# BUTSpeechFIT/VBx

Measured on NVIDIA H100. Metric: x-vectors/sec through 10 VB-HMM EM iters, higher is better.
Workload: dtype f32

## Files before the change

vbx_b200/csrc/vbx_kernels.cu:

```cuda
#include <math_constants.h>

#include "vbx_internal.cuh"

namespace vbx {

__device__ __forceinline__ void cp_async16(void *smem, const void *gmem) {
    unsigned s = static_cast<unsigned>(__cvta_generic_to_shared(smem));
    asm volatile("cp.async.cg.shared.global [%0], [%1], 16;\n" ::"r"(s), "l"(gmem));
}
__device__ __forceinline__ void cp_async_wait_all() {
    asm volatile("cp.async.commit_group;\n" ::);
    asm volatile("cp.async.wait_group 0;\n" ::: "memory");
}

template <int LANES>
__device__ __forceinline__ float group_sum(float v) {
#pragma unroll
    for (int off = LANES / 2; off > 0; off >>= 1) v += __shfl_xor_sync(0xffffffffu, v, off);
    return v;
}
template <int LANES>
__device__ __forceinline__ float group_max(float v) {
#pragma unroll
    for (int off = LANES / 2; off > 0; off >>= 1) v = fmaxf(v, __shfl_xor_sync(0xffffffffu, v, off));
// ... 324 lines not shown
    }
    const int R4 = R >> 2;
    float *out = ws.partial + (int64_t)tile * S_PAD * R;
    for (int i = threadIdx.x; i < S_PAD * R4; i += 256) {
        const int s = i / R4, c4 = i - s * R4;
        *reinterpret_cast<float4 *>(out + (int64_t)s * R + 4 * c4) = *reinterpret_cast<const float4 *>(&red[s][4 * c4]);
    }
}

int launch_mstep_partial(const Plan &pl, const Workspace &ws, const float *rho, const float *gamma, cudaStream_t st) {
    if (pl.n_mtiles == 0) return 0;
    switch (pl.S) {
        case 4: mstep_partial_kernel<4><<<pl.n_mtiles, 256, 0, st>>>(pl, ws, rho, gamma); break;
        case 8: mstep_partial_kernel<8><<<pl.n_mtiles, 256, 0, st>>>(pl, ws, rho, gamma); break;
        case 16: mstep_partial_kernel<16><<<pl.n_mtiles, 256, 0, st>>>(pl, ws, rho, gamma); break;
        case 32: mstep_partial_kernel<32><<<pl.n_mtiles, 256, 0, st>>>(pl, ws, rho, gamma); break;
        case 64: mstep_partial_kernel<64><<<pl.n_mtiles, 256, 0, st>>>(pl, ws, rho, gamma); break;
        case kMaxSWide: {
            constexpr int smem = kMaxSWide * kMaxR * sizeof(float);
            static bool configured = false;
            if (!configured) {
                if (cudaFuncSetAttribute(mstep_partial_kernel<kMaxSWide>, cudaFuncAttributeMaxDynamicSharedMemorySize, smem) != cudaSuccess)
                    return -1;
                configured = true;
            }
            mstep_partial_kernel<kMaxSWide><<<pl.n_mtiles, 256, smem, st>>>(pl, ws, rho, gamma);
            break;
        }
        default: return -1;
    }
    return cudaGetLastError() == cudaSuccess ? 1 : -1;
}

template <int S8, bool R128>
__global__ void __launch_bounds__(512) speaker_model_kernel(Plan pl, Workspace ws, const float *__restrict__ Phi,
                                                            const int32_t *__restrict__ n_states, float *alpha_io,
                                                            float *invL_io, int from_given) {
    const int S = pl.S, R = pl.R;
    constexpr int NT = S8 / 8, NSP = S8 / 4;
    const int rec = blockIdx.x;
    if (!ws.active[rec]) return;
    const float FaFb = ws.hp[rec].FaFb, Fa = ws.hp[rec].Fa;
    const int wg = threadIdx.x >> 7;
    const int r = threadIdx.x & 127, warp = r >> 5, lane = r & 31;
    const bool live = r < R;
    const int ns = n_states ? n_states[rec] : S;
    const float phi = live ? Phi[r] : 0.f;
    const int t_lo = pl.mtile_begin[rec], t_hi = pl.mtile_begin[rec + 1];
    extern __shared__ float sAv[];
    __shared__ double cpart[S8 > kMaxS ? S8 : kMaxS][4], rpart[S8 > kMaxS ? S8 : kMaxS][4];
    constexpr int NCH = NSP < 16 ? NSP : 16;
#pragma unroll
    for (int k0 = 0; k0 < NSP; k0 += NCH) {
    double grs[NCH];
#pragma unroll
    for (int k = 0; k < NCH; ++k) {
        const int s = wg + 4 * (k0 + k);
        double gr = 0.0;
        if (live && s < ns && !from_given)
            for (int t = t_lo; t < t_hi; ++t) gr += (double)__ldg(ws.partial + ((int64_t)t * S + s) * R + r);
        grs[k] = gr;
    }
#pragma unroll
    for (int k = 0; k < NCH; ++k) {
        const int s = wg + 4 * (k0 + k);
        const int64_t o = ((int64_t)rec * S + s) * R + r;
        const bool dead = s >= ns;
        float invL = 1.f, alpha = 0.f, Av = 0.f;
        float c = 0.f, reg = 0.f;
        if (live && !dead) {
            if (from_given) {
                alpha = alpha_io[o];
                invL = invL_io[o];
            } else {
                const double gr = grs[k];
                const float Ns = ws.occ[(int64_t)rec * S + s];
                invL = 1.f / (1.f + FaFb * Ns * phi);
                alpha = (float)((double)(FaFb * invL) * gr);
            }
            Av = Fa * alpha;
            const float a2 = alpha * alpha;
            reg = logf(invL) - invL - a2 + 1.f;
            c = (invL + a2) * phi;
        }
        if (live && s < S) {
            ws.A[o] = Av;
            if (!from_given || dead) {
                if (alpha_io) alpha_io[o] = dead ? 0.f : alpha;
                if (invL_io) invL_io[o] = dead ? 0.f : invL;
            }
        }
        sAv[s * kMaxR + r] = Av;
        c = group_sum<32>(c);
        reg = group_sum<32>(reg);
        if (lane == 0) {
            cpart[s][warp] = (double)c;
            rpart[s][warp] = (double)reg;
        }
    }
    }
    __syncthreads();
    if (threadIdx.x < S) {
        const int s = threadIdx.x;
        const bool dead = s >= ns;
        ws.bias[(int64_t)rec * S + s] =
            dead ? CUDART_INF_F : (float)(ws.hp[rec].dFa * 0.5 * ((cpart[s][0] + cpart[s][1]) + (cpart[s][2] + cpart[s][3])));
        ws.regp[(int64_t)rec * S + s] = dead ? 0.0 : (rpart[s][0] + rpart[s][1]) + (rpart[s][2] + rpart[s][3]);
    }
    const int KS = R128 ? 16 : (R + 7) >> 3, KQ = 2 * KS;
    float *fh = ws.Afrag_hi + (int64_t)rec * NT * KS * 64, *fl = ws.Afrag_lo + (int64_t)rec * NT * KS * 64;
    for (int q = threadIdx.x; q < NT * KS * 64; q += 512) {
        const int e = q & 1, ln = (q >> 1) & 31, ij = q >> 6;
        const int j = R128 ? (ij & 15) : ij % KS, i = R128 ? (ij >> 4) : ij / KS;
        const int st = 8 * i + (ln >> 2), fq = ln & 3;
        const int col = R128 ? 16 * (j >> 1) + 4 * fq + 2 * (j & 1) + e : KQ * fq + 2 * j + e;
        const float Av = col < kMaxR ? sAv[st * kMaxR + col] : 0.f;
        const float hi = __uint_as_float(__float_as_uint(Av) & 0xffffe000u);
        fh[q] = hi;
        fl[q] = Av - hi;
    }
}

int launch_speaker_model(const Plan &pl, const Workspace &ws, const float *Phi,
                         const int32_t *n_states, float *alpha_io, float *invL_io, bool from_given,
                         cudaStream_t st) {
    if (pl.n_rec == 0) return 0;
    const int S8 = pl.S > 8 ? pl.S : 8;
    const size_t smem = (size_t)S8 * kMaxR * sizeof(float);
    const int fg = from_given ? 1 : 0;
    if (S8 == kMaxSWide) {
        static bool configured = false;
        if (!configured) {
            if (cudaFuncSetAttribute(speaker_model_kernel<kMaxSWide, true>, cudaFuncAttributeMaxDynamicSharedMemorySize, (int)smem) != cudaSuccess ||
                cudaFuncSetAttribute(speaker_model_kernel<kMaxSWide, false>, cudaFuncAttributeMaxDynamicSharedMemorySize, (int)smem) != cudaSuccess)
                return -1;
            configured = true;
        }
    }
#define VBX_SM(S8_, R_) speaker_model_kernel<S8_, R_><<<pl.n_rec, 512, smem, st>>>(pl, ws, Phi, n_states, alpha_io, invL_io, fg)
    if (pl.R == 128) {
        switch (S8) {
            case 8: VBX_SM(8, true); break;
            case 16: VBX_SM(16, true); break;
            case 32: VBX_SM(32, true); break;
            case kMaxSWide: VBX_SM(kMaxSWide, true); break;
            default: VBX_SM(64, true); break;
        }
    } else {
        switch (S8) {
            case 8: VBX_SM(8, false); break;
            case 16: VBX_SM(16, false); break;
            case 32: VBX_SM(32, false); break;
            case kMaxSWide: VBX_SM(kMaxSWide, false); break;
            default: VBX_SM(64, false); break;
        }
    }
#undef VBX_SM
    return cudaGetLastError() == cudaSuccess ? 1 : -1;
}

template <int S_PAD>
__global__ void __launch_bounds__(128) loglik_kernel(Plan pl, Workspace ws, const float *__restrict__ rho,
                                                     const float *__restrict__ pi, const int32_t *__restrict__ n_states) {
    constexpr int SL = S_PAD < 8 ? S_PAD : 8;
    constexpr int SJ = S_PAD / SL;
    constexpr int FL = 128 / SL;
    constexpr int FJ = kLTile / FL;
    extern __shared__ float4 smem4[];
    float *smem = reinterpret_cast<float *>(smem4);
    const int R = pl.R, RP = R + 4, R4 = R >> 2;
    float *rhoS = smem;
    float *AS = smem + kLTile * RP;
    const int tile = blockIdx.x;
    const int rec = pl.ltile_rec[tile];
    if (!ws.active[rec]) return;
    const int64_t f0 = pl.ltile_f0[tile];
    const int len = (int)min((int64_t)kLTile, pl.offsets[rec + 1] - f0);
    const int tid = threadIdx.x;
    {
        const float *src = rho + f0 * R;
        for (int i = tid; i < len * R4; i += 128) {
            const int row = i / R4, c4 = i - row * R4;
            cp_async16(rhoS + row * RP + 4 * c4, src + (int64_t)row * R + 4 * c4);
        }
        const float *Ab = ws.A + (int64_t)rec * S_PAD * R;
        for (int i = tid; i < S_PAD * R4; i += 128) {
            const int row = i / R4, c4 = i - row * R4;
            cp_async16(AS + row * RP + 4 * c4, Ab + (int64_t)row * R + 4 * c4);
// ... 662 lines not shown
    for (int k = 0; k < SPL; ++k) {
        ys[k] = (st.rn * ps.v[k]) * fmaf(P, st.y[k], w[k] * st.Yc);
        locq = fmaf(pn.v[k], ys[k], locq);
        locc = fmaf(pn.v[k], w[k], locc);
    }
    const float qn = group_sum<LPR>(locq);
    const float cn = group_sum<LPR>(locc);
    const float Ys = st.rn * fmaf(P, st.q, st.c * st.Yc);
    const float inv = rcp_fast(Ys);
    const float rsig = st.rn * st.Yc * inv;
#pragma unroll
    for (int k = 0; k < SPL; ++k) {
        an[k] = ys[k] * inv;
        st.y[k] = ys[k];
    }
    st.Yc = Ys;
    st.q = qn;
    st.c = cn;
    st.rn = st.rs1;
    st.rs1 = rsig;
    return rsig;
}

template <int S_PAD, int SPL>
struct FbRing {
    static constexpr int LPR = S_PAD / SPL, RPW = 32 / LPR;
    static constexpr int F = (SPL == 4) ? 5 : (SPL == 2 ? 10 : 16);
    static constexpr int FF = 2 * F;
    static constexpr int RW = (F + 6 + 3) / 4 * 4;
    static constexpr int GROUP = 2 * F * S_PAD + RW;
    static constexpr int STAGE = RPW * GROUP;
    static constexpr int kStages = 3;
    static constexpr int kSmemBytes = 128 + 4 * kStages * STAGE * 4;
};

template <int S_PAD, int SPL>
__global__ void __launch_bounds__(128) forward_backward_ring_kernel(Plan pl, Workspace ws, RunParams rp, float *gamma,
                                                                    float *pi_io, const int32_t *__restrict__ n_states) {
    using G = FbRing<S_PAD, SPL>;
    constexpr int LPR = G::LPR, RPW = G::RPW, F = G::F, FF = G::FF, NST = G::kStages;
    extern __shared__ __align__(128) unsigned char fb_ring_smem[];
    const int lane = threadIdx.x & 31, warp = threadIdx.x >> 5;
    const int warp_global = blockIdx.x * 4 + warp;
    const int g = lane / LPR, l = lane % LPR;
    const int slot = warp_global * RPW + g;
    int rec = -1;
    if (slot < pl.n_rec) rec = pl.order[slot];
    const bool live = rec >= 0 && ws.active[rec] != 0 && pl.lrec_nchunks[rec] == 0;
    int64_t f0 = 0;
    int T = 0;
    if (live) {
        f0 = pl.offsets[rec];
        T = (int)(pl.offsets[rec + 1] - f0);
    }
    int Tmax = T, Tmin = live ? T : 0x7fffffff;
#pragma unroll
    for (int off = 16; off > 0; off >>= 1) {
        Tmax = max(Tmax, __shfl_xor_sync(0xffffffffu, Tmax, off));
        Tmin = min(Tmin, __shfl_xor_sync(0xffffffffu, Tmin, off));
    }
    if (Tmax == 0) return;
    const int Tlast = max(T - 1, 0);
    const int ns = live ? (n_states ? n_states[rec] : S_PAD) : 0;
    const float P = rec >= 0 ? ws.hp[rec].loopP : 0.f, Q = 1.f - P;

    float pi[SPL], w[SPL];
#pragma unroll
    for (int k = 0; k < SPL; ++k) {
        const int s = l * SPL + k;
        const bool sl = live && s < ns;
// ... 159 lines not shown
            }
            {
                const float sc = rcp_fast(group_sum<LPR>(gs));
#pragma unroll
                for (int k = 0; k < SPL; ++k) gn[k] *= sc;
            }
            if (!check) {
#pragma unroll
                for (int k = 0; k < SPL; ++k) {
                    g0[k] = gn[k];
                    occf[k] += gn[k];
                    entf[k] += v[k];
                }
                sto_vec<SPL>(ga + t * gstr, gn);
            } else {
                const bool act = t >= 0;
#pragma unroll
                for (int k = 0; k < SPL; ++k) {
                    g0[k] = act ? gn[k] : g0[k];
                    occf[k] += act ? gn[k] : 0.f;
                    entf[k] += act ? v[k] : 0.f;
                }
                if (act) sto_vec<SPL>(ga + t * gstr, gn);
            }
#pragma unroll
            for (int k = 0; k < SPL; ++k) {
                b[k] = bn[k];
                kap[k] = kapn[k];
            }
            dprev = d;
            e = en;
            f = fn;
        };
        auto bstage = [&](const int u, const float *st, const int rb, const bool check) {
            const float *sp = st + l * SPL, *sr = st + 2 * F * S_PAD;
            const int lo = T - 1 - (u + 1) * F, z = min(max(-lo, 0), F - 1);
            Vec<SPL> pr[F];
            float rt[F];
#pragma unroll
            for (int i = 0; i < F; ++i) {
                pr[i] = ld_vec<SPL>(sp + i * S_PAD);
                rt[i] = sr[max(rb - i, 0)];
            }
            FwdState<SPL> fs, f1;
            {
                const Vec<SPL> cy = ld_vec<SPL>(sp + F * S_PAD);
                const Vec<4> c4 = ld_vec<4>(st + (F + 1) * S_PAD);
                const float crs = st[(F + 2) * S_PAD];
                const Vec<SPL> q0 = ld_vec<SPL>(sp + z * S_PAD), q1 = ld_vec<SPL>(sp + min(z + 1, F - 1) * S_PAD);
                if (u + NST - 1 < nb) issue_bwd(u + NST - 1);
                float a0[SPL];
                fwd_init<SPL, LPR>(f1, q0, q1, pi, w, l, live, ns, a0);
                const bool ck = lo >= 1;
#pragma unroll
                for (int k = 0; k < SPL; ++k) {
                    fs.y[k] = ck ? cy.v[k] : f1.y[k];
                    f1.y[k] = a0[k];
                }
                fs.Yc = ck ? c4.v[0] : f1.Yc;
                fs.q = ck ? c4.v[1] : f1.q;
                fs.c = ck ? c4.v[2] : f1.c;
                fs.rn = ck ? c4.v[3] : f1.rn;
                fs.rs1 = ck ? crs : f1.rs1;
            }
            Vec<SPL> a[F];
#pragma unroll
            for (int i = 0; i < F; ++i) {
                const int s = lo + i;
                FwdState<SPL> nx = fs;
                fwd_step<SPL, LPR>(nx, pr[i], pr[min(i + 1, F - 1)], w, P, a[i].v);
                if (s >= 1) fs = nx;
#pragma unroll
                for (int k = 0; k < SPL; ++k) a[i].v[k] = s == 0 ? f1.y[k] : a[i].v[k];
            }
#pragma unroll
            for (int i = 0; i < F; ++i) bstep(u * F + i, a[F - 1 - i], pr[F - 1 - i], rt[i], check);
#pragma unroll
            for (int k = 0; k < SPL; ++k) {
                occ[k] += (double)occf[k];
                enter[k] += (double)entf[k];
                occf[k] = 0.f;
                entf[k] = 0.f;
            }
        };
        for (int u = 0; u < nb; ++u) {
            mbar_wait(bar_of(nf + u), ((nf + u) / NST) & 1);
            const float *st = stage_of(nf + u);
            const int rb = (int)min((int64_t)(T - 2 - u * F) - rwin(u), (int64_t)(G::RW - 1));
            if ((u + 1) * F <= Tmin - 1)
                bstage(u, st, rb, false);
            else
                bstage(u, st, rb, true);
        }
    }

    double pn[SPL];
    float loc = 0.f;
#pragma unroll
    for (int k = 0; k < SPL; ++k) {
        pn[k] = (double)g0[k] + (double)Q * (double)pi[k] * enter[k];
        loc += (float)pn[k];
    }
    const float tot = group_sum<LPR>(loc);
    if (live) {
#pragma unroll
        for (int k = 0; k < SPL; ++k) {
            const int s = l * SPL + k;
            pi_io[(int64_t)rec * S_PAD + s] = (float)(pn[k] / (double)tot);
            ws.occ[(int64_t)rec * S_PAD + s] = (float)occ[k];
        }
    }
}

constexpr int64_t kRingMaxT = 2048;

template <int S_PAD, int SPL>
static int launch_fb_t(const Plan &pl, const Workspace &ws, const RunParams &rp, float *gamma, float *pi,
                       const int32_t *n_states, bool classic, bool ring, cudaStream_t st) {
    constexpr int RPW = 32 / (S_PAD / SPL);
    const int warps = (pl.n_rec + RPW - 1) / RPW;
    const int blocks = (warps + 3) / 4;
    if (classic) {
        forward_backward_kernel<S_PAD, SPL><<<blocks, 128, 0, st>>>(pl, ws, rp, gamma, pi, n_states);
    } else if (ring && pl.max_T <= kRingMaxT && (reinterpret_cast<uintptr_t>(gamma) & 15) == 0) {
        constexpr int smem = FbRing<S_PAD, SPL>::kSmemBytes;
        if (cudaFuncSetAttribute(forward_backward_ring_kernel<S_PAD, SPL>, cudaFuncAttributeMaxDynamicSharedMemorySize,
                                 smem) != cudaSuccess)
            return -1;
        forward_backward_ring_kernel<S_PAD, SPL><<<blocks, 128, smem, st>>>(pl, ws, rp, gamma, pi, n_states);
    } else {
        forward_backward_la_kernel<S_PAD, SPL><<<blocks, 128, 0, st>>>(pl, ws, rp, gamma, pi, n_states);
    }
    return cudaGetLastError() == cudaSuccess ? 1 : -1;
}

__global__ void __launch_bounds__(128) elbo_kernel(Plan pl, Workspace ws, RunParams rp, double *Li, int32_t *n_iters,
                                                   int32_t *flags, int iter) {
    const int rec = blockIdx.x;
    if (!ws.active[rec]) return;
    const int tid = threadIdx.x, lane = tid & 31, warp = tid >> 5;
    const int64_t f0 = pl.offsets[rec];
    const int T = (int)(pl.offsets[rec + 1] - f0);
    const float *rs = ws.rsigma + f0;
    const float *mx = ws.rowmax + f0;
    double acc = 0.0;
    for (int t = tid; t < T; t += 128) acc += (double)mx[t] - log((double)rs[t]);
    acc = warp_sum_d(acc);
// ... 124 lines not shown
```

vbx_b200/csrc/vbx_capi.cu:

```cuda
#include <dlfcn.h>
#include <nvtx3/nvToolsExt.h>

#include <algorithm>
#include <cmath>
#include <cstdio>
#include <cstring>
#include <numeric>
#include <string>
#include <vector>

#include "../../include/vbx_b200.h"
#include "vbx_internal.cuh"

struct vbx_handle_s {
    int device = 0;
    int sms = 0;
    std::string err;
    vbx::Plan plan;
    vbx::Workspace ws;
    bool planned = false, bound = false, prepared = false;
    bool f64_only = false;
    size_t ws_need = 0;
    void *plan_mem = nullptr;
    int opt_fb_spl = 0;
// ... 56 lines not shown
    }
    DeviceGuard(const DeviceGuard &) = delete;
    DeviceGuard &operator=(const DeviceGuard &) = delete;
};

struct Carver {
    char *base;
    size_t off = 0;
    explicit Carver(void *b) : base(static_cast<char *>(b)) {}
    template <typename T>
    T *take(size_t n) {
        T *p = base ? reinterpret_cast<T *>(base + off) : nullptr;
        off += align_up(n * sizeof(T));
        return p;
    }
};

void drop_graph(vbx_handle_t h) {
    if (h->graph_exec) cudaGraphExecDestroy(h->graph_exec);
    h->graph_exec = nullptr;
    h->graph_key = h->seen_key = 0;
}

size_t carve(const vbx::Plan &pl, void *base, vbx::Workspace *ws) {
    Carver c(base);
    const size_t N = (size_t)pl.n_frames, S = (size_t)pl.S, R = (size_t)pl.R, B = (size_t)pl.n_rec;
    vbx::Workspace w;
    w.p = c.take<float>(N * S);
    w.rowmax = c.take<float>(N);
    w.rsigma = c.take<float>(N);
    w.cvec = c.take<float>(N);
    w.partial = c.take<float>((size_t)pl.n_mtiles * S * R);
    w.A = c.take<float>(B * S * R);
    {
        const size_t NT = S > 8 ? S / 8 : 1, KS = (R + 7) / 8;
        w.Afrag_hi = c.take<float>(B * NT * KS * 64);
        w.Afrag_lo = c.take<float>(B * NT * KS * 64);
    }
    w.bias = c.take<float>(B * S);
    w.occ = c.take<float>(B * S);
    w.regp = c.take<double>(B * S);
    w.gsum = c.take<double>(B);
    w.gpart = c.take<double>((size_t)pl.n_mtiles);
    w.prev_elbo = c.take<double>(B);
    w.active = c.take<int32_t>(B);
    w.scratch = c.take<float>(2 * std::max<size_t>(S, vbx::kMaxS));
    if (pl.R == 128) w.tc_scratch = c.take<float>(vbx::tc_scratch_floats());
    if (pl.split) {
        w.ahat = c.take<float>(N * S);
        w.bhat = c.take<float>(N * S);
        w.socc = c.take<float>((size_t)pl.n_mtiles * S);
        w.sent = c.take<float>((size_t)pl.n_mtiles * S);
    }
    {
        const size_t LC = (size_t)pl.n_lchunks;
        w.fa_u = c.take<float>(LC * S * S);
        w.fa_lam = c.take<float>(LC * S);
        w.fa_exp = c.take<float>(LC * S);
        w.astart = c.take<float>(LC * S);
        w.bb_v = c.take<float>(LC * S * S);
        w.bb_mu = c.take<float>(LC * S);
        w.bb_exp = c.take<float>(LC * S);
        w.beta = c.take<float>(LC * S);
        w.occp = c.take<float>(LC * S);
        w.entp = c.take<float>(LC * S);
    }
    if (pl.exact) {
        w.active64 = c.take<int32_t>(B);
        w.fresh = c.take<int32_t>(B);
        w.gamma_snap = c.take<float>(2 * N * S);
        w.pi_snap = c.take<float>(2 * B * S);
// ... 1136 lines not shown
```

vbx_b200/csrc/vbx_internal.cuh:

```cuda
#pragma once
#include <cuda_runtime.h>
#include <stdint.h>

#include <string>
#include <vector>

#define VBX_EPS_TR 1e-8f

namespace vbx {

constexpr int kLTile = 64;
constexpr int kMTile = 512;
constexpr int kLongT = 4096;
constexpr int kChunk = 256;
constexpr int kMaxR = 128;
constexpr int kMaxS = 64;
constexpr int kMaxSWide = 128;
constexpr int kTcMaxD = 2048;

struct Plan {
    int32_t n_rec = 0, R = 0, S = 0;
    int32_t exact = 0;
    int32_t split = 0;
    int64_t n_frames = 0;
    int32_t n_ltiles = 0, n_mtiles = 0;
    int64_t max_T = 0;
    const int64_t *offsets = nullptr;
    const int32_t *order = nullptr;
    const int32_t *ltile_rec = nullptr;
    const int64_t *ltile_f0 = nullptr;
    const int32_t *mtile_rec = nullptr;
    const int64_t *mtile_f0 = nullptr;
    const int32_t *mtile_begin = nullptr;
    int32_t n_lrec = 0, n_lchunks = 0;
    const int32_t *lrec_list = nullptr;
    const int32_t *lrec_first = nullptr;
    const int32_t *lrec_nchunks = nullptr;
    const int32_t *lchunk_rec = nullptr;
    const int32_t *lchunk_idx = nullptr;
};

struct RecParams {
    float Fa, Fb, FaFb, loopP;
    double dFa, dFb, dFaFb, dloopP;
};

struct Workspace {
    float *p = nullptr;
    float *rowmax = nullptr;
    float *rsigma = nullptr;
    float *cvec = nullptr;
    float *partial = nullptr;
    float *A = nullptr;
    float *Afrag_hi = nullptr;
    float *Afrag_lo = nullptr;
    float *bias = nullptr;
    float *occ = nullptr;
    double *regp = nullptr;
    double *gsum = nullptr;
    double *gpart = nullptr;
    double *prev_elbo = nullptr;
    int32_t *active = nullptr;
    int32_t *active64 = nullptr;
    int32_t *fresh = nullptr;
    float *gamma_snap = nullptr;
    float *pi_snap = nullptr;
    double *p64 = nullptr;
    double *rowmax64 = nullptr;
    double *rsig64 = nullptr;
    double *partial64 = nullptr;
    double *occp64 = nullptr;
    double *alpha64 = nullptr;
    double *bias64 = nullptr;
    double *reg64 = nullptr;
    double *pi64 = nullptr;
    float *scratch = nullptr;
    float *ahat = nullptr, *bhat = nullptr;
    float *socc = nullptr, *sent = nullptr;
    float *tc_scratch = nullptr;
    float *fa_u = nullptr, *fa_lam = nullptr, *fa_exp = nullptr, *astart = nullptr;
    float *bb_v = nullptr, *bb_mu = nullptr, *bb_exp = nullptr, *beta = nullptr;
    float *occp = nullptr, *entp = nullptr;
    RecParams *hp = nullptr;
};

struct RunParams {
    double epsilon;
    int32_t max_iters;
// ... 242 lines not shown
```

vbx_b200/csrc/vbx_mma_kernels.cu:

```cuda
#include <math_constants.h>

#include "vbx_internal.cuh"

namespace vbx {

__device__ __forceinline__ void mma_tf32(float (&d)[4], const uint32_t (&a)[4], const uint32_t b0, const uint32_t b1) {
    asm volatile(
        "mma.sync.aligned.m16n8k8.row.col.f32.tf32.tf32.f32 {%0,%1,%2,%3}, {%4,%5,%6,%7}, {%8,%9}, {%0,%1,%2,%3};\n"
        : "+f"(d[0]), "+f"(d[1]), "+f"(d[2]), "+f"(d[3])
        : "r"(a[0]), "r"(a[1]), "r"(a[2]), "r"(a[3]), "r"(b0), "r"(b1));
}
__device__ __forceinline__ void split_tf32(const float x, uint32_t &hi, uint32_t &lo) {
    asm volatile("{\n\t.reg .b32 t;\n\tadd.u32 t, %1, 0x1000;\n\tand.b32 %0, t, 0xffffe000;\n\t}" : "=r"(hi) : "r"(__float_as_uint(x)));
    lo = (__float_as_uint(x - __uint_as_float(hi)) + 0x1000u) & 0xffffe000u;
}
__device__ __forceinline__ void cp_async16_(void *smem, const void *gmem) {
    unsigned s = static_cast<unsigned>(__cvta_generic_to_shared(smem));
    asm volatile("cp.async.cg.shared.global [%0], [%1], 16;\n" ::"r"(s), "l"(gmem));
}

template <int S_PAD>
__global__ void __launch_bounds__(S_PAD > kMaxS ? 256 : 128, S_PAD > kMaxS ? 2 : 4)
    mstep_mma_kernel(Plan pl, Workspace ws, const float *__restrict__ rho, const float *__restrict__ gamma) {
    constexpr int SH = S_PAD > kMaxS ? S_PAD / kMaxS : 1;
    constexpr int SB = S_PAD / SH;
    constexpr int MT = SB > 16 ? SB / 16 : 1;
    constexpr int NTW = 16 / MT;
    constexpr int RW = 8 * NTW;
    constexpr int FS = 4 / MT;
    constexpr int NQ = NTW / 4;
    constexpr int S16 = 16 * MT;
    constexpr int LD = kMaxR + 4;
    __shared__ __align__(16) float red_st[SH > 1 ? 1 : FS][SH > 1 ? 1 : S16][LD];
    extern __shared__ float4 red_dyn[];
    float (*red)[S16 * SH][LD] = SH > 1 ? reinterpret_cast<float (*)[S16 * SH][LD]>(red_dyn) : reinterpret_cast<float (*)[S16 * SH][LD]>(red_st);
    const int tile = blockIdx.x;
    const int rec = pl.mtile_rec[tile];
    if (!ws.active[rec]) return;
    const int64_t f0 = pl.mtile_f0[tile];
    const int len = (int)min((int64_t)kMTile, pl.offsets[rec + 1] - f0);
    const int warp = threadIdx.x >> 5, lane = threadIdx.x & 31;
    const int g = lane >> 2, q = lane & 3;
    const int sh = SH > 1 ? warp >> 2 : 0, w4 = SH > 1 ? (warp & 3) : warp;
    const int rg = w4 % MT, fs = w4 / MT;
    const int R = pl.R;
    const int col0 = rg * RW + 4 * g;
    const float *grow = gamma + f0 * S_PAD + sh * SB;

    float acc[MT][NTW][4];
#pragma unroll
    for (int m = 0; m < MT; ++m)
// ... 101 lines not shown
            static bool configured = false;
            if (!configured) {
                if (cudaFuncSetAttribute(mstep_mma_kernel<kMaxSWide>, cudaFuncAttributeMaxDynamicSharedMemorySize, smem) != cudaSuccess)
                    return -1;
                configured = true;
            }
            mstep_mma_kernel<kMaxSWide><<<pl.n_mtiles, 256, smem, st>>>(pl, ws, rho, gamma);
            break;
        }
        default: return -1;
    }
    return cudaGetLastError() == cudaSuccess ? 1 : -1;
}

template <int S_PAD, bool R128, bool WITH_C>
__global__ void __launch_bounds__(S_PAD > kMaxS ? 256 : 128, S_PAD > kMaxS ? 1 : 3)
    loglik_mma_kernel(Plan pl, Workspace ws, const float *__restrict__ rho, const float *__restrict__ pi,
                      const int32_t *__restrict__ n_states) {
    constexpr int NT = S_PAD > 8 ? S_PAD / 8 : 1;
    constexpr int NW = S_PAD > kMaxS ? 8 : 4;
    constexpr bool SPLIT_E = S_PAD <= kMaxS;
    extern __shared__ uint2 sfrag[];
    const int R = pl.R;
    const int KS = R128 ? 16 : (R + 7) >> 3;
    const int KQ = 2 * KS;
    uint2 *sBh = sfrag, *sBl = sfrag + NT * KS * 32;
    const int tile = blockIdx.x;
    const int rec = pl.mtile_rec[tile];
    if (!ws.active[rec]) return;
    const int64_t f0 = pl.mtile_f0[tile];
    const int len = (int)min((int64_t)kMTile, pl.offsets[rec + 1] - f0);
    const int tid = threadIdx.x, warp = tid >> 5, lane = tid & 31;
    const int g = lane >> 2, q = lane & 3;
    {
        const int n16 = NT * KS * 32 / 2;
        const uint4 *gh = reinterpret_cast<const uint4 *>(ws.Afrag_hi + (int64_t)rec * NT * KS * 64);
        const uint4 *gl = reinterpret_cast<const uint4 *>(ws.Afrag_lo + (int64_t)rec * NT * KS * 64);
        for (int i = tid; i < n16; i += 32 * NW) {
            cp_async16_(reinterpret_cast<uint4 *>(sBh) + i, gh + i);
            cp_async16_(reinterpret_cast<uint4 *>(sBl) + i, gl + i);
        }
        asm volatile("cp.async.commit_group;\n" ::);
    }
    float nb[NT][2], wv[NT][2];
    const int ns = n_states ? n_states[rec] : S_PAD;
    const float Q = WITH_C ? 1.f - ws.hp[rec].loopP : 0.f;
#pragma unroll
    for (int i = 0; i < NT; ++i) {
        const int s = 8 * i + 2 * q;
        nb[i][0] = s < S_PAD ? -ws.bias[(int64_t)rec * S_PAD + s] : -CUDART_INF_F;
        nb[i][1] = s + 1 < S_PAD ? -ws.bias[(int64_t)rec * S_PAD + s + 1] : -CUDART_INF_F;
        wv[i][0] = (WITH_C && s < ns) ? fmaf(Q, pi[(int64_t)rec * S_PAD + s], VBX_EPS_TR) : 0.f;
        wv[i][1] = (WITH_C && s + 1 < ns) ? fmaf(Q, pi[(int64_t)rec * S_PAD + s + 1], VBX_EPS_TR) : 0.f;
    }
    const int n_mt = (len + 15) >> 4;

    auto finish = [&](float (&D)[NT][4], const float (&E)[NT][4], const int mt) {
        if constexpr (SPLIT_E) {
#pragma unroll
            for (int i = 0; i < NT; ++i)
#pragma unroll
                for (int e = 0; e < 4; ++e) D[i][e] += E[i][e];
        }
        float m0 = fmaxf(D[0][0], D[0][1]), m1 = fmaxf(D[0][2], D[0][3]);
#pragma unroll
        for (int i = 1; i < NT; ++i) {
            m0 = fmaxf(m0, fmaxf(D[i][0], D[i][1]));
            m1 = fmaxf(m1, fmaxf(D[i][2], D[i][3]));
        }
        m0 = fmaxf(m0, __shfl_xor_sync(0xffffffffu, m0, 1));
        m1 = fmaxf(m1, __shfl_xor_sync(0xffffffffu, m1, 1));
        m0 = fmaxf(m0, __shfl_xor_sync(0xffffffffu, m0, 2));
        m1 = fmaxf(m1, __shfl_xor_sync(0xffffffffu, m1, 2));
        const int ra = mt * 16 + g, rb = ra + 8;
        float c0 = 0.f, c1 = 0.f;
#pragma unroll
// ... 53 lines not shown
    if (R128 && SPLIT_E) {
        struct Raw {
            float4 xa[8], xb[8];
        };
        auto load_mt = [&](const int mt, Raw &r) {
            const int ra = min(mt * 16 + g, len - 1), rb = min(mt * 16 + g + 8, len - 1);
            const float4 *pa = reinterpret_cast<const float4 *>(rho + (f0 + ra) * 128 + 4 * q);
            const float4 *pb = reinterpret_cast<const float4 *>(rho + (f0 + rb) * 128 + 4 * q);
#pragma unroll
            for (int k = 0; k < 8; ++k) {
                r.xa[k] = __ldg(pa + 4 * k);
                r.xb[k] = __ldg(pb + 4 * k);
            }
        };
        auto compute = [&](const Raw &r, const int mt) {
            float D[NT][4], E[NT][4];
#pragma unroll
            for (int i = 0; i < NT; ++i) {
                D[i][0] = nb[i][0];
                D[i][1] = nb[i][1];
                D[i][2] = nb[i][0];
                D[i][3] = nb[i][1];
                E[i][0] = E[i][1] = E[i][2] = E[i][3] = 0.f;
            }
#pragma unroll
            for (int k = 0; k < 8; ++k) {
                kstep(D, E, 2 * k, r.xa[k].x, r.xb[k].x, r.xa[k].y, r.xb[k].y);
                kstep(D, E, 2 * k + 1, r.xa[k].z, r.xb[k].z, r.xa[k].w, r.xb[k].w);
            }
            finish(D, E, mt);
        };
        Raw r0;
        load_mt(warp, r0);
        asm volatile("cp.async.wait_group 0;\n" ::: "memory");
        __syncthreads();
        for (int mt = warp; mt < n_mt; mt += NW) {
            if (mt != warp) load_mt(mt, r0);
            compute(r0, mt);
        }
    } else {
        asm volatile("cp.async.wait_group 0;\n" ::: "memory");
        __syncthreads();
        for (int mt = warp; mt < n_mt; mt += NW) {
            float D[NT][4], E[NT][4];
#pragma unroll
            for (int i = 0; i < NT; ++i) {
                D[i][0] = nb[i][0];
                D[i][1] = nb[i][1];
                D[i][2] = nb[i][0];
                D[i][3] = nb[i][1];
                E[i][0] = E[i][1] = E[i][2] = E[i][3] = 0.f;
            }
            const int ra = min(mt * 16 + g, len - 1), rb = min(mt * 16 + g + 8, len - 1);
            const float *pa = rho + (f0 + ra) * R;
            const float *pb = rho + (f0 + rb) * R;
#pragma unroll 4
            for (int j = 0; j < KS; ++j) {
                const int col = R128 ? 16 * (j >> 1) + 4 * q + 2 * (j & 1) : KQ * q + 2 * j;
                const int cc = min(col, R - 2);
                const float2 va = __ldg(reinterpret_cast<const float2 *>(pa + cc));
                const float2 vb = __ldg(reinterpret_cast<const float2 *>(pb + cc));
                kstep(D, E, j, va.x, vb.x, va.y, vb.y);
            }
            finish(D, E, mt);
        }
    }
}

static size_t loglik_mma_smem(int S_pad, int R) {
    const int NT = S_pad > 8 ? S_pad / 8 : 1, KS = (R + 7) / 8;
    return (size_t)2 * NT * KS * 32 * sizeof(uint2);
}

template <int S_PAD>
// ... 60 lines not shown
```

Measured before the change: 172.4 million.

## Software-pipeline backward pass by recomputing next block's forward while stepping current

Restructures the backward ring loop so that the forward recomputation for block u+1 is interleaved with the backward steps of block u, with state carried in double-buffered register arrays. The goal is to expose instruction-level parallelism between two independent dependency chains, and to skip the init/check logic on interior blocks where no boundary checks are needed. It is enabled only for certain S_PAD/SPL configurations, and the extra register arrays raise register pressure and may cause spills.

```diff
diff --git a/vbx_b200/csrc/vbx_kernels.cu b/vbx_b200/csrc/vbx_kernels.cu
--- a/vbx_b200/csrc/vbx_kernels.cu
+++ b/vbx_b200/csrc/vbx_kernels.cu
@@ -1230,6 +1230,7 @@
     static constexpr int STAGE = RPW * GROUP;
     static constexpr int kStages = 3;
     static constexpr int kSmemBytes = 128 + 4 * kStages * STAGE * 4;
+    static constexpr bool kPipelined = SPL != 4 && !(S_PAD == 32 && SPL == 1);
 };
 
 template <int S_PAD, int SPL>
@@ -1459,49 +1460,72 @@
             e = en;
             f = fn;
         };
-        auto bstage = [&](const int u, const float *st, const int rb, const bool check) {
-            const float *sp = st + l * SPL, *sr = st + 2 * F * S_PAD;
-            const int lo = T - 1 - (u + 1) * F, z = min(max(-lo, 0), F - 1);
-            Vec<SPL> pr[F];
-            float rt[F];
+        Vec<SPL> pc[F], ac[F], pn[F], an[F];
+        float rc[F], rn[F], a0[SPL];
+        FwdState<SPL> fs;
+        int lon = 0;
+        auto load_next = [&](const int v, const bool rcheck) {
+            const float *st = stage_of(nf + v), *sp = st + l * SPL, *sr = st + 2 * F * S_PAD;
+            const int rb = (int)min((int64_t)(T - 2 - v * F) - rwin(v), (int64_t)(G::RW - 1));
+            lon = T - 1 - (v + 1) * F;
+            const int z = min(max(-lon, 0), F - 1);
 #pragma unroll
             for (int i = 0; i < F; ++i) {
-                pr[i] = ld_vec<SPL>(sp + i * S_PAD);
-                rt[i] = sr[max(rb - i, 0)];
-            }
-            FwdState<SPL> fs, f1;
-            {
-                const Vec<SPL> cy = ld_vec<SPL>(sp + F * S_PAD);
-                const Vec<4> c4 = ld_vec<4>(st + (F + 1) * S_PAD);
-                const float crs = st[(F + 2) * S_PAD];
-                const Vec<SPL> q0 = ld_vec<SPL>(sp + z * S_PAD), q1 = ld_vec<SPL>(sp + min(z + 1, F - 1) * S_PAD);
-                if (u + NST - 1 < nb) issue_bwd(u + NST - 1);
-                float a0[SPL];
+                pn[i] = ld_vec<SPL>(sp + i * S_PAD);
+                rn[i] = sr[max(rb - i, 0)];
+            }
+            const Vec<SPL> cy = ld_vec<SPL>(sp + F * S_PAD);
+            const Vec<4> c4 = ld_vec<4>(st + (F + 1) * S_PAD);
+            const float crs = st[(F + 2) * S_PAD];
+            const Vec<SPL> q0 = ld_vec<SPL>(sp + z * S_PAD), q1 = ld_vec<SPL>(sp + min(z + 1, F - 1) * S_PAD);
+            if (v + NST - 1 < nb) issue_bwd(v + NST - 1);
+            if (!rcheck) {
+#pragma unroll
+                for (int k = 0; k < SPL; ++k) fs.y[k] = cy.v[k];
+                fs.Yc = c4.v[0];
+                fs.q = c4.v[1];
+                fs.c = c4.v[2];
+                fs.rn = c4.v[3];
+                fs.rs1 = crs;
+            } else {
+                FwdState<SPL> f1;
                 fwd_init<SPL, LPR>(f1, q0, q1, pi, w, l, live, ns, a0);
-                const bool ck = lo >= 1;
-#pragma unroll
-                for (int k = 0; k < SPL; ++k) {
-                    fs.y[k] = ck ? cy.v[k] : f1.y[k];
-                    f1.y[k] = a0[k];
-                }
+                const bool ck = lon >= 1;
+#pragma unroll
+                for (int k = 0; k < SPL; ++k) fs.y[k] = ck ? cy.v[k] : f1.y[k];
                 fs.Yc = ck ? c4.v[0] : f1.Yc;
                 fs.q = ck ? c4.v[1] : f1.q;
                 fs.c = ck ? c4.v[2] : f1.c;
                 fs.rn = ck ? c4.v[3] : f1.rn;
                 fs.rs1 = ck ? crs : f1.rs1;
             }
-            Vec<SPL> a[F];
+        };
+        auto rstep = [&](const int i, const bool rcheck) {
+            const int s = lon + i;
+            FwdState<SPL> nx = fs;
+            fwd_step<SPL, LPR>(nx, pn[i], pn[min(i + 1, F - 1)], w, P, an[i].v);
+            if (!rcheck || s >= 1) fs = nx;
+            if (rcheck) {
+#pragma unroll
+                for (int k = 0; k < SPL; ++k) an[i].v[k] = s == 0 ? a0[k] : an[i].v[k];
+            }
+        };
+        auto bstage = [&](const int u, const bool check, const bool ahead) {
 #pragma unroll
             for (int i = 0; i < F; ++i) {
-                const int s = lo + i;
-                FwdState<SPL> nx = fs;
-                fwd_step<SPL, LPR>(nx, pr[i], pr[min(i + 1, F - 1)], w, P, a[i].v);
-                if (s >= 1) fs = nx;
-#pragma unroll
-                for (int k = 0; k < SPL; ++k) a[i].v[k] = s == 0 ? f1.y[k] : a[i].v[k];
-            }
-#pragma unroll
-            for (int i = 0; i < F; ++i) bstep(u * F + i, a[F - 1 - i], pr[F - 1 - i], rt[i], check);
+                pc[i] = pn[i];
+                ac[i] = an[i];
+                rc[i] = rn[i];
+            }
+            if (ahead) {
+                mbar_wait(bar_of(nf + u + 1), ((nf + u + 1) / NST) & 1);
+                load_next(u + 1, check);
+            }
+#pragma unroll
+            for (int i = 0; i < F; ++i) {
+                bstep(u * F + i, ac[F - 1 - i], pc[F - 1 - i], rc[i], check);
+                if (ahead) rstep(i, check);
+            }
 #pragma unroll
             for (int k = 0; k < SPL; ++k) {
                 occ[k] += (double)occf[k];
@@ -1510,14 +1534,32 @@
                 entf[k] = 0.f;
             }
         };
-        for (int u = 0; u < nb; ++u) {
-            mbar_wait(bar_of(nf + u), ((nf + u) / NST) & 1);
-            const float *st = stage_of(nf + u);
-            const int rb = (int)min((int64_t)(T - 2 - u * F) - rwin(u), (int64_t)(G::RW - 1));
-            if ((u + 1) * F <= Tmin - 1)
-                bstage(u, st, rb, false);
-            else
-                bstage(u, st, rb, true);
+        if constexpr (!G::kPipelined) {
+            for (int u = 0; u < nb; ++u) {
+                mbar_wait(bar_of(nf + u), ((nf + u) / NST) & 1);
+                load_next(u, true);
+#pragma unroll
+                for (int i = 0; i < F; ++i) rstep(i, true);
+                if ((u + 1) * F <= Tmin - 1)
+                    bstage(u, false, false);
+                else
+                    bstage(u, true, false);
+            }
+        } else {
+            if (nb > 0) {
+                mbar_wait(bar_of(nf), (nf / NST) & 1);
+                load_next(0, true);
+#pragma unroll
+                for (int i = 0; i < F; ++i) rstep(i, true);
+            }
+            for (int u = 0; u < nb; ++u) {
+                if (u + 1 == nb)
+                    bstage(u, true, false);
+                else if ((u + 2) * F <= Tmin - 2)
+                    bstage(u, false, true);
+                else
+                    bstage(u, true, true);
+            }
         }
     }
 
```

After: 172.7 million, median of 6. About the same (+0.2%).

## Build TF32 hi/lo fragments in the E-step kernel instead of storing them globally

Applied to the files above, without the earlier changes.

The speaker-model kernel no longer writes the precomputed hi/lo TF32 fragment arrays through shared memory. Each E-step tile now reads the speaker matrix A and splits it into fragments straight into shared memory. The partial-sum reduction is also restructured to batch loads across time tiles, occupancy hints are added to launch bounds, and occ values are staged in shared memory. This removes a global write/read round trip and the speaker kernel's large dynamic shared memory, at the cost of recomputing the split in every E-step tile.

```diff
diff --git a/vbx_b200/csrc/vbx_capi.cu b/vbx_b200/csrc/vbx_capi.cu
--- a/vbx_b200/csrc/vbx_capi.cu
+++ b/vbx_b200/csrc/vbx_capi.cu
@@ -112,11 +112,6 @@
     w.cvec = c.take<float>(N);
     w.partial = c.take<float>((size_t)pl.n_mtiles * S * R);
     w.A = c.take<float>(B * S * R);
-    {
-        const size_t NT = S > 8 ? S / 8 : 1, KS = (R + 7) / 8;
-        w.Afrag_hi = c.take<float>(B * NT * KS * 64);
-        w.Afrag_lo = c.take<float>(B * NT * KS * 64);
-    }
     w.bias = c.take<float>(B * S);
     w.occ = c.take<float>(B * S);
     w.regp = c.take<double>(B * S);
diff --git a/vbx_b200/csrc/vbx_internal.cuh b/vbx_b200/csrc/vbx_internal.cuh
--- a/vbx_b200/csrc/vbx_internal.cuh
+++ b/vbx_b200/csrc/vbx_internal.cuh
@@ -52,8 +52,6 @@
     float *cvec = nullptr;
     float *partial = nullptr;
     float *A = nullptr;
-    float *Afrag_hi = nullptr;
-    float *Afrag_lo = nullptr;
     float *bias = nullptr;
     float *occ = nullptr;
     double *regp = nullptr;
diff --git a/vbx_b200/csrc/vbx_kernels.cu b/vbx_b200/csrc/vbx_kernels.cu
--- a/vbx_b200/csrc/vbx_kernels.cu
+++ b/vbx_b200/csrc/vbx_kernels.cu
@@ -380,35 +380,53 @@
     return cudaGetLastError() == cudaSuccess ? 1 : -1;
 }
 
-template <int S8, bool R128>
-__global__ void __launch_bounds__(512) speaker_model_kernel(Plan pl, Workspace ws, const float *__restrict__ Phi,
+template <int S8>
+__global__ void __launch_bounds__(512, S8 <= 16 ? 3 : 2) speaker_model_kernel(Plan pl, Workspace ws, const float *__restrict__ Phi,
                                                             const int32_t *__restrict__ n_states, float *alpha_io,
                                                             float *invL_io, int from_given) {
     const int S = pl.S, R = pl.R;
-    constexpr int NT = S8 / 8, NSP = S8 / 4;
+    constexpr int NSP = S8 / 4;
     const int rec = blockIdx.x;
     if (!ws.active[rec]) return;
     const float FaFb = ws.hp[rec].FaFb, Fa = ws.hp[rec].Fa;
+    const double dFa = ws.hp[rec].dFa;
     const int wg = threadIdx.x >> 7;
     const int r = threadIdx.x & 127, warp = r >> 5, lane = r & 31;
     const bool live = r < R;
     const int ns = n_states ? n_states[rec] : S;
     const float phi = live ? Phi[r] : 0.f;
     const int t_lo = pl.mtile_begin[rec], t_hi = pl.mtile_begin[rec + 1];
-    extern __shared__ float sAv[];
     __shared__ double cpart[S8 > kMaxS ? S8 : kMaxS][4], rpart[S8 > kMaxS ? S8 : kMaxS][4];
-    constexpr int NCH = NSP < 16 ? NSP : 16;
+    __shared__ float socc[S8];
+    if (!from_given && threadIdx.x < S) socc[threadIdx.x] = ws.occ[(int64_t)rec * S + threadIdx.x];
+    constexpr int NCH = NSP < 8 ? NSP : 8;
+    constexpr int TB = NCH < 4 ? 4 : 2;
 #pragma unroll
     for (int k0 = 0; k0 < NSP; k0 += NCH) {
     double grs[NCH];
 #pragma unroll
-    for (int k = 0; k < NCH; ++k) {
-        const int s = wg + 4 * (k0 + k);
-        double gr = 0.0;
-        if (live && s < ns && !from_given)
-            for (int t = t_lo; t < t_hi; ++t) gr += (double)__ldg(ws.partial + ((int64_t)t * S + s) * R + r);
-        grs[k] = gr;
-    }
+    for (int k = 0; k < NCH; ++k) grs[k] = 0.0;
+    if (live && !from_given) {
+        const float *prow = ws.partial + ((int64_t)t_lo * S + wg + 4 * k0) * R + r;
+#pragma unroll 1
+        for (int t0 = 0; t0 < t_hi - t_lo; t0 += TB, prow += TB * S * R) {
+            float v[NCH][TB];
+#pragma unroll
+            for (int k = 0; k < NCH; ++k) {
+                const int s = wg + 4 * (k0 + k);
+#pragma unroll
+                for (int u = 0; u < TB; ++u) {
+                    v[k][u] = 0.f;
+                    if (s < ns && t0 + u < t_hi - t_lo) v[k][u] = __ldg(prow + (u * S + 4 * k) * R);
+                }
+            }
+#pragma unroll
+            for (int k = 0; k < NCH; ++k)
+#pragma unroll
+                for (int u = 0; u < TB; ++u) grs[k] += (double)v[k][u];
+        }
+    }
+    if (k0 == 0) __syncthreads();
 #pragma unroll
     for (int k = 0; k < NCH; ++k) {
         const int s = wg + 4 * (k0 + k);
@@ -422,7 +440,7 @@
                 invL = invL_io[o];
             } else {
                 const double gr = grs[k];
-                const float Ns = ws.occ[(int64_t)rec * S + s];
+                const float Ns = socc[s];
                 invL = 1.f / (1.f + FaFb * Ns * phi);
                 alpha = (float)((double)(FaFb * invL) * gr);
             }
@@ -438,7 +456,6 @@
                 if (invL_io) invL_io[o] = dead ? 0.f : invL;
             }
         }
-        sAv[s * kMaxR + r] = Av;
         c = group_sum<32>(c);
         reg = group_sum<32>(reg);
         if (lane == 0) {
@@ -452,20 +469,8 @@
         const int s = threadIdx.x;
         const bool dead = s >= ns;
         ws.bias[(int64_t)rec * S + s] =
-            dead ? CUDART_INF_F : (float)(ws.hp[rec].dFa * 0.5 * ((cpart[s][0] + cpart[s][1]) + (cpart[s][2] + cpart[s][3])));
+            dead ? CUDART_INF_F : (float)(dFa * 0.5 * ((cpart[s][0] + cpart[s][1]) + (cpart[s][2] + cpart[s][3])));
         ws.regp[(int64_t)rec * S + s] = dead ? 0.0 : (rpart[s][0] + rpart[s][1]) + (rpart[s][2] + rpart[s][3]);
-    }
-    const int KS = R128 ? 16 : (R + 7) >> 3, KQ = 2 * KS;
-    float *fh = ws.Afrag_hi + (int64_t)rec * NT * KS * 64, *fl = ws.Afrag_lo + (int64_t)rec * NT * KS * 64;
-    for (int q = threadIdx.x; q < NT * KS * 64; q += 512) {
-        const int e = q & 1, ln = (q >> 1) & 31, ij = q >> 6;
-        const int j = R128 ? (ij & 15) : ij % KS, i = R128 ? (ij >> 4) : ij / KS;
-        const int st = 8 * i + (ln >> 2), fq = ln & 3;
-        const int col = R128 ? 16 * (j >> 1) + 4 * fq + 2 * (j & 1) + e : KQ * fq + 2 * j + e;
-        const float Av = col < kMaxR ? sAv[st * kMaxR + col] : 0.f;
-        const float hi = __uint_as_float(__float_as_uint(Av) & 0xffffe000u);
-        fh[q] = hi;
-        fl[q] = Av - hi;
     }
 }
 
@@ -473,35 +478,14 @@
                          const int32_t *n_states, float *alpha_io, float *invL_io, bool from_given,
                          cudaStream_t st) {
     if (pl.n_rec == 0) return 0;
-    const int S8 = pl.S > 8 ? pl.S : 8;
-    const size_t smem = (size_t)S8 * kMaxR * sizeof(float);
     const int fg = from_given ? 1 : 0;
-    if (S8 == kMaxSWide) {
-        static bool configured = false;
-        if (!configured) {
-            if (cudaFuncSetAttribute(speaker_model_kernel<kMaxSWide, true>, cudaFuncAttributeMaxDynamicSharedMemorySize, (int)smem) != cudaSuccess ||
-                cudaFuncSetAttribute(speaker_model_kernel<kMaxSWide, false>, cudaFuncAttributeMaxDynamicSharedMemorySize, (int)smem) != cudaSuccess)
-                return -1;
-            configured = true;
-        }
-    }
-#define VBX_SM(S8_, R_) speaker_model_kernel<S8_, R_><<<pl.n_rec, 512, smem, st>>>(pl, ws, Phi, n_states, alpha_io, invL_io, fg)
-    if (pl.R == 128) {
-        switch (S8) {
-            case 8: VBX_SM(8, true); break;
-            case 16: VBX_SM(16, true); break;
-            case 32: VBX_SM(32, true); break;
-            case kMaxSWide: VBX_SM(kMaxSWide, true); break;
-            default: VBX_SM(64, true); break;
-        }
-    } else {
-        switch (S8) {
-            case 8: VBX_SM(8, false); break;
-            case 16: VBX_SM(16, false); break;
-            case 32: VBX_SM(32, false); break;
-            case kMaxSWide: VBX_SM(kMaxSWide, false); break;
-            default: VBX_SM(64, false); break;
-        }
+#define VBX_SM(S8_) speaker_model_kernel<S8_><<<pl.n_rec, 512, 0, st>>>(pl, ws, Phi, n_states, alpha_io, invL_io, fg)
+    switch (pl.S > 8 ? pl.S : 8) {
+        case 8: VBX_SM(8); break;
+        case 16: VBX_SM(16); break;
+        case 32: VBX_SM(32); break;
+        case kMaxSWide: VBX_SM(kMaxSWide); break;
+        default: VBX_SM(64); break;
     }
 #undef VBX_SM
     return cudaGetLastError() == cudaSuccess ? 1 : -1;
diff --git a/vbx_b200/csrc/vbx_mma_kernels.cu b/vbx_b200/csrc/vbx_mma_kernels.cu
--- a/vbx_b200/csrc/vbx_mma_kernels.cu
+++ b/vbx_b200/csrc/vbx_mma_kernels.cu
@@ -13,10 +13,6 @@
 __device__ __forceinline__ void split_tf32(const float x, uint32_t &hi, uint32_t &lo) {
     asm volatile("{\n\t.reg .b32 t;\n\tadd.u32 t, %1, 0x1000;\n\tand.b32 %0, t, 0xffffe000;\n\t}" : "=r"(hi) : "r"(__float_as_uint(x)));
     lo = (__float_as_uint(x - __uint_as_float(hi)) + 0x1000u) & 0xffffe000u;
-}
-__device__ __forceinline__ void cp_async16_(void *smem, const void *gmem) {
-    unsigned s = static_cast<unsigned>(__cvta_generic_to_shared(smem));
-    asm volatile("cp.async.cg.shared.global [%0], [%1], 16;\n" ::"r"(s), "l"(gmem));
 }
 
 template <int S_PAD>
@@ -184,16 +180,26 @@
     const int len = (int)min((int64_t)kMTile, pl.offsets[rec + 1] - f0);
     const int tid = threadIdx.x, warp = tid >> 5, lane = tid & 31;
     const int g = lane >> 2, q = lane & 3;
-    {
-        const int n16 = NT * KS * 32 / 2;
-        const uint4 *gh = reinterpret_cast<const uint4 *>(ws.Afrag_hi + (int64_t)rec * NT * KS * 64);
-        const uint4 *gl = reinterpret_cast<const uint4 *>(ws.Afrag_lo + (int64_t)rec * NT * KS * 64);
-        for (int i = tid; i < n16; i += 32 * NW) {
-            cp_async16_(reinterpret_cast<uint4 *>(sBh) + i, gh + i);
-            cp_async16_(reinterpret_cast<uint4 *>(sBl) + i, gl + i);
-        }
-        asm volatile("cp.async.commit_group;\n" ::);
-    }
+    auto build_frags = [&]() {
+        const float *A = ws.A + (int64_t)rec * S_PAD * R;
+        auto one = [&](const int idx) {
+            const int ln = idx & 31, ij = idx >> 5;
+            const int j = R128 ? (ij & 15) : ij % KS, i = R128 ? (ij >> 4) : ij / KS;
+            const int st = 8 * i + (ln >> 2), fq = ln & 3;
+            const int col = R128 ? 16 * (j >> 1) + 4 * fq + 2 * (j & 1) : KQ * fq + 2 * j;
+            float2 av = make_float2(0.f, 0.f);
+            if (st < S_PAD && col < R) av = __ldg(reinterpret_cast<const float2 *>(A + st * R + col));
+            const uint32_t h0 = __float_as_uint(av.x) & 0xffffe000u, h1 = __float_as_uint(av.y) & 0xffffe000u;
+            sBh[idx] = make_uint2(h0, h1);
+            sBl[idx] = make_uint2(__float_as_uint(av.x - __uint_as_float(h0)), __float_as_uint(av.y - __uint_as_float(h1)));
+        };
+        if constexpr (R128) {
+#pragma unroll
+            for (int k = 0; k < NT * 16 * 32 / (32 * NW); ++k) one(tid + 32 * NW * k);
+        } else {
+            for (int idx = tid; idx < NT * KS * 32; idx += 32 * NW) one(idx);
+        }
+    };
     float nb[NT][2], wv[NT][2];
     const int ns = n_states ? n_states[rec] : S_PAD;
     const float Q = WITH_C ? 1.f - ws.hp[rec].loopP : 0.f;
@@ -313,14 +319,14 @@
         };
         Raw r0;
         load_mt(warp, r0);
-        asm volatile("cp.async.wait_group 0;\n" ::: "memory");
+        build_frags();
         __syncthreads();
         for (int mt = warp; mt < n_mt; mt += NW) {
             if (mt != warp) load_mt(mt, r0);
             compute(r0, mt);
         }
     } else {
-        asm volatile("cp.async.wait_group 0;\n" ::: "memory");
+        build_frags();
         __syncthreads();
         for (int mt = warp; mt < n_mt; mt += NW) {
             float D[NT][4], E[NT][4];
```

After: 172.3 million before, 176.0 million after (median of 6 runs). 2.2% higher.

## Software-pipeline ring backward pass: recompute next stage's forward while backward-stepping current

Applied to the files above, without the earlier changes.

The backward pass of the ring forward-backward kernel now loads stage u+1 and interleaves its forward recomputation steps with the backward steps of stage u. This exposes two independent dependency chains so latency can overlap instead of running serially. It also sets launch bounds to 2 blocks per SM and raises the maximum T allowed for the ring path to 4095. The cost is higher register pressure from the doubled stage arrays, which the occupancy hint may turn into spills.

```diff
diff --git a/vbx_b200/csrc/vbx_kernels.cu b/vbx_b200/csrc/vbx_kernels.cu
--- a/vbx_b200/csrc/vbx_kernels.cu
+++ b/vbx_b200/csrc/vbx_kernels.cu
@@ -1230,10 +1230,11 @@
     static constexpr int STAGE = RPW * GROUP;
     static constexpr int kStages = 3;
     static constexpr int kSmemBytes = 128 + 4 * kStages * STAGE * 4;
+    static_assert(4 * kStages * 8 <= 128, "the mbarriers of the 4 warps fit in front of the rings");
 };
 
 template <int S_PAD, int SPL>
-__global__ void __launch_bounds__(128) forward_backward_ring_kernel(Plan pl, Workspace ws, RunParams rp, float *gamma,
+__global__ void __launch_bounds__(128, 2) forward_backward_ring_kernel(Plan pl, Workspace ws, RunParams rp, float *gamma,
                                                                     float *pi_io, const int32_t *__restrict__ n_states) {
     using G = FbRing<S_PAD, SPL>;
     constexpr int LPR = G::LPR, RPW = G::RPW, F = G::F, FF = G::FF, NST = G::kStages;
@@ -1459,49 +1460,51 @@
             e = en;
             f = fn;
         };
-        auto bstage = [&](const int u, const float *st, const int rb, const bool check) {
-            const float *sp = st + l * SPL, *sr = st + 2 * F * S_PAD;
+        auto load_stage = [&](const int u, Vec<SPL>(&pr)[F], float(&rt)[F], FwdState<SPL> &fs, float(&a0)[SPL]) {
+            mbar_wait(bar_of(nf + u), ((nf + u) / NST) & 1);
+            const float *st = stage_of(nf + u), *sp = st + l * SPL, *sr = st + 2 * F * S_PAD;
+            const int rb = (int)min((int64_t)(T - 2 - u * F) - rwin(u), (int64_t)(G::RW - 1));
             const int lo = T - 1 - (u + 1) * F, z = min(max(-lo, 0), F - 1);
-            Vec<SPL> pr[F];
-            float rt[F];
 #pragma unroll
             for (int i = 0; i < F; ++i) {
                 pr[i] = ld_vec<SPL>(sp + i * S_PAD);
                 rt[i] = sr[max(rb - i, 0)];
             }
-            FwdState<SPL> fs, f1;
-            {
-                const Vec<SPL> cy = ld_vec<SPL>(sp + F * S_PAD);
-                const Vec<4> c4 = ld_vec<4>(st + (F + 1) * S_PAD);
-                const float crs = st[(F + 2) * S_PAD];
-                const Vec<SPL> q0 = ld_vec<SPL>(sp + z * S_PAD), q1 = ld_vec<SPL>(sp + min(z + 1, F - 1) * S_PAD);
-                if (u + NST - 1 < nb) issue_bwd(u + NST - 1);
-                float a0[SPL];
-                fwd_init<SPL, LPR>(f1, q0, q1, pi, w, l, live, ns, a0);
-                const bool ck = lo >= 1;
-#pragma unroll
-                for (int k = 0; k < SPL; ++k) {
-                    fs.y[k] = ck ? cy.v[k] : f1.y[k];
-                    f1.y[k] = a0[k];
-                }
-                fs.Yc = ck ? c4.v[0] : f1.Yc;
-                fs.q = ck ? c4.v[1] : f1.q;
-                fs.c = ck ? c4.v[2] : f1.c;
-                fs.rn = ck ? c4.v[3] : f1.rn;
-                fs.rs1 = ck ? crs : f1.rs1;
-            }
-            Vec<SPL> a[F];
+            const Vec<SPL> cy = ld_vec<SPL>(sp + F * S_PAD);
+            const Vec<4> c4 = ld_vec<4>(st + (F + 1) * S_PAD);
+            const float crs = st[(F + 2) * S_PAD];
+            const Vec<SPL> q0 = ld_vec<SPL>(sp + z * S_PAD), q1 = ld_vec<SPL>(sp + min(z + 1, F - 1) * S_PAD);
+            if (u + NST - 1 < nb) issue_bwd(u + NST - 1);
+            FwdState<SPL> f1;
+            fwd_init<SPL, LPR>(f1, q0, q1, pi, w, l, live, ns, a0);
+            const bool ck = lo >= 1;
+#pragma unroll
+            for (int k = 0; k < SPL; ++k) fs.y[k] = ck ? cy.v[k] : f1.y[k];
+            fs.Yc = ck ? c4.v[0] : f1.Yc;
+            fs.q = ck ? c4.v[1] : f1.q;
+            fs.c = ck ? c4.v[2] : f1.c;
+            fs.rn = ck ? c4.v[3] : f1.rn;
+            fs.rs1 = ck ? crs : f1.rs1;
+        };
+        auto rstep = [&](const int s, const int i, FwdState<SPL> &fs, const Vec<SPL>(&pr)[F], const float(&a0)[SPL],
+                         Vec<SPL> &a) {
+            FwdState<SPL> nx = fs;
+            fwd_step<SPL, LPR>(nx, pr[i], pr[min(i + 1, F - 1)], w, P, a.v);
+            if (s >= 1) fs = nx;
+#pragma unroll
+            for (int k = 0; k < SPL; ++k) a.v[k] = s == 0 ? a0[k] : a.v[k];
+        };
+        Vec<SPL> pr[F], a[F], pn[F], an[F];
+        float rt[F], rn[F];
+        FwdState<SPL> fs;
+        float a0[SPL];
+        auto bstage = [&](const int u, const bool next, const bool check) {
+            const int lo = T - 1 - (u + 2) * F;
 #pragma unroll
             for (int i = 0; i < F; ++i) {
-                const int s = lo + i;
-                FwdState<SPL> nx = fs;
-                fwd_step<SPL, LPR>(nx, pr[i], pr[min(i + 1, F - 1)], w, P, a[i].v);
-                if (s >= 1) fs = nx;
-#pragma unroll
-                for (int k = 0; k < SPL; ++k) a[i].v[k] = s == 0 ? f1.y[k] : a[i].v[k];
-            }
-#pragma unroll
-            for (int i = 0; i < F; ++i) bstep(u * F + i, a[F - 1 - i], pr[F - 1 - i], rt[i], check);
+                if (next) rstep(lo + i, i, fs, pn, a0, an[i]);
+                bstep(u * F + i, a[F - 1 - i], pr[F - 1 - i], rt[i], check);
+            }
 #pragma unroll
             for (int k = 0; k < SPL; ++k) {
                 occ[k] += (double)occf[k];
@@ -1510,14 +1513,30 @@
                 entf[k] = 0.f;
             }
         };
+        if (nb > 0) {
+            load_stage(0, pr, rt, fs, a0);
+#pragma unroll
+            for (int i = 0; i < F; ++i) rstep(T - 1 - F + i, i, fs, pr, a0, a[i]);
+        }
         for (int u = 0; u < nb; ++u) {
-            mbar_wait(bar_of(nf + u), ((nf + u) / NST) & 1);
-            const float *st = stage_of(nf + u);
-            const int rb = (int)min((int64_t)(T - 2 - u * F) - rwin(u), (int64_t)(G::RW - 1));
-            if ((u + 1) * F <= Tmin - 1)
-                bstage(u, st, rb, false);
-            else
-                bstage(u, st, rb, true);
+            const bool check = (u + 1) * F > Tmin - 1;
+            if (u + 1 < nb) {
+                load_stage(u + 1, pn, rn, fs, a0);
+                if (!check)
+                    bstage(u, true, false);
+                else
+                    bstage(u, true, true);
+#pragma unroll
+                for (int i = 0; i < F; ++i) {
+                    pr[i] = pn[i];
+                    a[i] = an[i];
+                    rt[i] = rn[i];
+                }
+            } else if (!check) {
+                bstage(u, false, false);
+            } else {
+                bstage(u, false, true);
+            }
         }
     }
 
@@ -1539,7 +1558,7 @@
     }
 }
 
-constexpr int64_t kRingMaxT = 2048;
+constexpr int64_t kRingMaxT = 4095;
 
 template <int S_PAD, int SPL>
 static int launch_fb_t(const Plan &pl, const Workspace &ws, const RunParams &rp, float *gamma, float *pi,
```

New measurement: 172.3 million before, 173.9 million after, median of 6. No clear change (+1.0%).
